# Scalsol/mega.pytorch

Hardware: AMD Instinct MI355X
Metric: frames/sec MEGA R-101 inference, 1000x600 VID clip (higher is better)
Workload: dtype bf16

## Files before the change

mega/pytorch_amd/build.py:

```python
import hashlib
import os
import subprocess
import sys

HERE = os.path.dirname(os.path.abspath(__file__))
CSRC = os.path.join(HERE, "csrc")
LIB = os.path.join(HERE, "libmega_hip.so")
STAMP = os.path.join(HERE, "csrc", ".build_stamp")
SOURCES = {
    "igemm.hip": [],
    "igemm8.hip": [],
    "igemm4.hip": [],
    "igemm2.hip": [],
    "stream1x1.hip": [],
    "spatial.hip": [],
    "boxes.hip": ["-ffp-contract=off"],
    "relation.hip": ["-mllvm", "-amdgpu-mfma-vgpr-form=1"],
    "frames.hip": ["-ffp-contract=off"],
    "fgfa.hip": [],
    "assemble.hip": [],
    "conv64.hip": [],
    "bneck64.hip": [],
    "vid_eval.hip": ["-ffp-contract=off"],
    "seq_nms.hip": ["-ffp-contract=off"],
}
HIPCC = os.environ.get("HIPCC", "/opt/rocm/bin/hipcc")
BASE_FLAGS = ["--offload-arch=gfx950", "-O3", "-std=c++17", "-fPIC", "-Wno-unused-result"]
if os.environ.get("MEGA_BUILD_EXPERIMENTS") == "1":
    BASE_FLAGS.append("-DMEGA_EXPERIMENTS")


def _probe_flags(flags):
    if not flags or not os.path.exists(HIPCC):
        return list(flags)
    import tempfile
    with tempfile.TemporaryDirectory() as td:
        src = os.path.join(td, "probe.hip")
        with open(src, "w") as f:
            f.write("#include <hip/hip_runtime.h>\n__global__ void mega_probe() {}\n")
        cmd = [HIPCC, "--offload-arch=gfx950", "-O1"] + list(flags) + ["-c", src, "-o", os.path.join(td, "probe.o")]
        if subprocess.run(cmd, stdout=subprocess.PIPE, stderr=subprocess.STDOUT).returncode == 0:
            return list(flags)
    sys.stderr.write("build.py: hipcc rejects %s -- building without it\n" % " ".join(flags))
    return []


def _digest():
    h = hashlib.sha256()
    for fn in sorted(os.listdir(CSRC)):
        if fn.endswith((".hip", ".h")):
            h.update(fn.encode())
            h.update(open(os.path.join(CSRC, fn), "rb").read())
    h.update(" ".join(BASE_FLAGS).encode())
    h.update(repr(sorted(SOURCES.items())).encode())
    h.update(open(os.path.abspath(__file__), "rb").read())
    return h.hexdigest()


def build(force=False, verbose=False):
    dig = _digest()
    if not force and os.path.exists(LIB) and os.path.exists(STAMP) and open(STAMP).read().strip() == dig:
        return LIB
    if not os.path.exists(HIPCC):
        if os.path.exists(LIB):
            return LIB
        raise RuntimeError("hipcc not found at %s and no prebuilt %s" % (HIPCC, LIB))
    objs = []
    procs = []
    for src, extra in SOURCES.items():
        path = os.path.join(CSRC, src)
        if not os.path.exists(path):
            continue
        if "-mllvm" in extra:
            extra = _probe_flags(extra)
        obj = os.path.join(CSRC, src.replace(".hip", ".o"))
        cmd = [HIPCC] + BASE_FLAGS + extra + ["-c", path, "-o", obj]
        if verbose:
            print(" ".join(cmd))
        procs.append((src, subprocess.Popen(cmd, stdout=subprocess.PIPE, stderr=subprocess.STDOUT)))
        objs.append(obj)
    for src, pr in procs:
        out, _ = pr.communicate()
        if pr.returncode != 0:
            raise RuntimeError("hipcc failed on %s:\n%s" % (src, out.decode()))
        if verbose and out:
            print(out.decode())
    cmd = [HIPCC, "--offload-arch=gfx950", "-shared", "-fPIC", "-o", LIB] + objs
    subprocess.check_call(cmd)
    with open(STAMP, "w") as f:
        f.write(dig)
    return LIB


if __name__ == "__main__":
    print(build(force="--force" in sys.argv, verbose=True))
```

mega/pytorch_amd/csrc/igemm.hip:

```cpp
#include <cstdio>
#include <cstdlib>

#include "common.h"
#include "igemm_params.h"

namespace {

constexpr int KTB = 128;
constexpr int LDS_STRIDE = 144;
constexpr int NTHREADS = 256;

template <typename T> struct Mma;
template <> struct Mma<bf16_t> {
  __device__ static __forceinline__ void run(f32x16_t& acc, const uint4& a, const uint4& b) {
    bf16x8_t av = __builtin_bit_cast(bf16x8_t, a);
    bf16x8_t bv = __builtin_bit_cast(bf16x8_t, b);
    acc = __builtin_amdgcn_mfma_f32_32x32x16_bf16(av, bv, acc, 0, 0, 0);
  }
};
template <> struct Mma<f16_t> {
  __device__ static __forceinline__ void run(f32x16_t& acc, const uint4& a, const uint4& b) {
    acc = __builtin_amdgcn_mfma_f32_32x32x16_f16(__builtin_bit_cast(f16x8_t, a), __builtin_bit_cast(f16x8_t, b), acc, 0, 0, 0);
  }
};
// ... 235 lines not shown
        asm volatile("" ::: "memory");
#pragma unroll
        for (int it = 0; it < NIT; ++it) {
          const int row = row0 + it * RSTEP;
          float v[OVE];
#pragma unroll
          for (int t = 0; t < OVE; t += 4) {
            const float4 f = *reinterpret_cast<const float4*>(cs + row * CST + cvo + t);
            v[t] = f.x; v[t + 1] = f.y; v[t + 2] = f.z; v[t + 3] = f.w;
          }
          if (HAS_RES) {
            const T* re = reinterpret_cast<const T*>(&rr[i % PD][it]);
#pragma unroll
            for (int t = 0; t < OVE; ++t) v[t] += Elem<T>::ld(re + t);
          }
          u32x4_t o;
          if constexpr (sizeof(OT) == 2) {
#pragma unroll
            for (int d = 0; d < 4; ++d) {
              if constexpr (RELU) {
                const s16x2_t z = {0, 0};
                o[d] = __builtin_bit_cast(unsigned, __builtin_elementwise_max(__builtin_bit_cast(s16x2_t, Half16<OT>::pack2(v[2 * d], v[2 * d + 1])), z));
              } else {
                o[d] = Half16<OT>::pack2(act(v[2 * d]), act(v[2 * d + 1]));
              }
            }
          } else {
#pragma unroll
            for (int t = 0; t < 4; ++t) o[t] = __float_as_uint(RELU ? fmaxf(v[t], 0.f) : act(v[t]));
          }
          __builtin_amdgcn_raw_buffer_store_b128(o, rs_out, out_off(slab_m(i, it)), 0, 0);
        }
        if (HAS_RES && i + PD < TM) ldres(i + PD, rr[i % PD]);
      }
    };
    if (res) {
      if (p.relu == 1) run(std::integral_constant<bool, RES_FAST>{}, std::true_type{});
      else run(std::integral_constant<bool, RES_FAST>{}, std::false_type{});
    } else {
      if (p.relu == 1) run(std::false_type{}, std::true_type{}); else run(std::false_type{}, std::false_type{});
    }
    return;
  }
  if (PS && p.ksplit == 1) return;
#pragma unroll
  for (int i = 0; i < TM; ++i) {
    if (i > 0) __syncthreads();
#pragma unroll
    for (int j = 0; j < TN; ++j) {
      const int nl = wn * WTN + j * 32 + (lane & 31);
      const int rb = wm * 32 + 4 * (lane >> 5);
#pragma unroll
      for (int r = 0; r < 16; ++r) cs[(rb + (r & 3) + 8 * (r >> 2)) * CST + nl] = acc[i][j][r] * sc[j] + bi[j];
    }
    __syncthreads();
    if (p.ksplit > 1) {
      float* part = p.partial + (size_t)blockIdx.z * p.M * p.Cout;
      for (int e = tid; e < 64 * (BN / 4); e += NTHREADS) {
        const int row = e / (BN / 4), cv = e - row * (BN / 4);
        const int m = m0 + (row >> 5) * WTM + i * 32 + (row & 31), n = n0 + cv * 4;
        if (m >= p.M || n >= p.Cout) continue;
        const float4 f = *reinterpret_cast<const float4*>(cs + row * CST + cv * 4);
        if (n + 4 <= p.Cout && p.Cout % 4 == 0) {
          *reinterpret_cast<float4*>(part + (size_t)m * p.Cout + n) = f;
        } else {
          const float v[4] = {f.x, f.y, f.z, f.w};
          for (int t = 0; t < 4 && n + t < p.Cout; ++t) part[(size_t)m * p.Cout + n + t] = v[t];
        }
      }
      continue;
    }
    for (int e = tid; e < 64 * VPR; e += NTHREADS) {
      const int row = e / VPR, cv = e - row * VPR;
      const int m = m0 + (row >> 5) * WTM + i * 32 + (row & 31), n = n0 + cv * OVE;
      if (m >= p.M || n >= p.Cout) continue;
      float v[OVE];
#pragma unroll
      for (int t = 0; t < OVE; t += 4) {
        const float4 f = *reinterpret_cast<const float4*>(cs + row * CST + cv * OVE + t);
        v[t] = f.x; v[t + 1] = f.y; v[t + 2] = f.z; v[t + 3] = f.w;
      }
      if (vec_ok && n + OVE <= p.Cout) {
        if (res) {
          const uint4 rr = *reinterpret_cast<const uint4*>(res + (size_t)m * p.ldr + n);
          const T* re = reinterpret_cast<const T*>(&rr);
#pragma unroll
          for (int t = 0; t < OVE; ++t) v[t] += Elem<T>::ld(re + t);
        }
        uint4 o;
        OT* oe = reinterpret_cast<OT*>(&o);
#pragma unroll
        for (int t = 0; t < OVE; ++t) Elem<OT>::st(oe + t, act(v[t]));
        *reinterpret_cast<uint4*>(out + (size_t)m * p.ldo + n) = o;
      } else {
        for (int t = 0; t < OVE && n + t < p.Cout; ++t) {
          float x = v[t];
          if (res) x += Elem<T>::ld(res + (size_t)m * p.ldr + n + t);
          x = act(x);
          Elem<OT>::st(out + (size_t)m * p.ldo + n + t, x);
        }
      }
    }
  }
}

template <typename T, typename OT, int BM, int BN, bool PS = false>
int launch(const ConvParams& p, hipStream_t st) {
  const int ntm = cdiv(p.M, BM), ntn = cdiv(p.Cout, BN);
  const size_t smem = 2 * (BM + BN) * LDS_STRIDE;
  (void)hipFuncSetAttribute((const void*)igemm_kernel<T, OT, BM, BN, PS>, hipFuncAttributeMaxDynamicSharedMemorySize, (int)smem);
  hipLaunchKernelGGL((igemm_kernel<T, OT, BM, BN, PS>), dim3(ntm * ntn, 1, p.ksplit), dim3(NTHREADS), smem, st, p);
  return mega_check_launch();
}

template <typename T, typename OT>
__global__ __launch_bounds__(256) void splitk_finalize_kernel(ConvParams p) {
  const size_t total = (size_t)p.M * p.Cout;
  const float neg_slope = p.relu == 1 ? 0.f : (p.relu == 2 ? 0.1f : 1.f);
  for (size_t i = (size_t)blockIdx.x * blockDim.x + threadIdx.x; i < total; i += (size_t)gridDim.x * blockDim.x) {
    const int m = (int)(i / p.Cout), n = (int)(i - (size_t)m * p.Cout);
    float v = 0.f;
    for (int z = 0; z < p.ksplit; ++z) v += p.partial[(size_t)z * total + i];
    v = v * (p.scale ? p.scale[n] : 1.f) + (p.bias ? p.bias[n] : 0.f);
    if (p.res) v += Elem<T>::ld((const T*)p.res + (size_t)m * p.ldr + n);
    v = v > 0.f ? v : v * neg_slope;
    if (p.ps) {
      const int HoWo = p.Ho * p.Wo, t = m / HoWo, rem = m - t * HoWo, mh = rem / p.Wo, mw = rem - mh * p.Wo;
      const int q = n / p.ps_C, y = 2 * mh + (q >> 1) - p.ps_crop, x = 2 * mw + (q & 1) - p.ps_crop;
      if ((unsigned)y < (unsigned)p.ps_H && (unsigned)x < (unsigned)p.ps_W)
        Elem<OT>::st((OT*)p.out + ((size_t)(t * p.ps_H + y) * p.ps_W + x) * p.ldo + p.ps_coff + (n - q * p.ps_C), v);
      continue;
    }
    Elem<OT>::st((OT*)p.out + (size_t)m * p.ldo + n, v);
  }
}

template <typename T, typename OT>
int launch_finalize(const ConvParams& p, hipStream_t st) {
  const size_t total = (size_t)p.M * p.Cout;
  const unsigned blocks = (unsigned)((total + 255) / 256 > 8192 ? 8192 : (total + 255) / 256);
  hipLaunchKernelGGL((splitk_finalize_kernel<T, OT>), dim3(blocks), dim3(256), 0, st, p);
  return mega_check_launch();
}

inline int choose_ksplit(int K) { return K >= 32768 ? 3 : 1; }

inline void choose_tile(int M, int Cout, int K, int z, bool bf16, int& kind, int& bm, int& bn) {
  kind = 0;
  const char* force = getenv("MEGA_IGEMM_TILE");
  if (force && sscanf(force, "8:%d", &bm) == 1) { kind = 8; bn = 256; return; }
  if (force && sscanf(force, "4:%d", &bm) == 1) { kind = 4; bn = 256; return; }
  if (force && sscanf(force, "2:%d", &bm) == 1) { kind = 2; bm = 128; bn = 256; return; }
  if (force && sscanf(force, "s:%d", &bm) == 1) { kind = 1; bm = 32; bn = 256; return; }
  if (force && sscanf(force, "%dx%d", &bm, &bn) == 2) return;
  const long b256 = (long)cdiv(M, 256) * cdiv(Cout, 256) * z;
  const long b128 = (long)cdiv(M, 128) * cdiv(Cout, 128) * z;
  const long b12864 = (long)cdiv(M, 128) * cdiv(Cout, 64) * z;
  static const int use8 = getenv("MEGA_IGEMM8") ? atoi(getenv("MEGA_IGEMM8")) : 1;
  static const int min_kt = getenv("MEGA_IGEMM8_MIN_KTILES") ? atoi(getenv("MEGA_IGEMM8_MIN_KTILES")) : 1;
  if (bf16 && use8 && Cout >= 256 && K >= 64 * min_kt) {
    const long t256 = (long)cdiv(M, 256) * cdiv(Cout, 256) * z, t192 = (long)cdiv(M, 192) * cdiv(Cout, 256) * z;
    const long c256 = cdiv((int)t256, 256) * 256L * 8, c192 = cdiv((int)t192, 256) * 192L * 9;
    if (t256 >= 128 || t192 >= 128) {
      kind = 8; bn = 256; bm = c192 < c256 ? 192 : 256;
      return;
    }
  }
  if (K >= 8192 && Cout >= 1024 && b256 >= 700) { bm = 256; bn = 256; }
  else if (Cout > 64 && b128 >= 384) { bm = 128; bn = 128; }
  else if (b12864 >= 384) { bm = 128; bn = 64; }
  else { bm = 64; bn = 64; }
}

template <typename T, typename OT>
int dispatch_tile(const ConvParams& p, hipStream_t st) {
  int kind = 0, bm = 0, bn = 0, rc;
  constexpr bool is_bf16 = sizeof(T) == 2;
  choose_tile(p.M, p.Cout, p.K, p.ksplit, is_bf16, kind, bm, bn);
  if (kind == 8 && !(is_bf16 && mega_igemm8_supports(p))) {
    kind = 0; bm = 128; bn = 128;
  }
  if constexpr (is_bf16 && sizeof(OT) == 2) {
    static const int use_s = getenv("MEGA_STREAM1X1") ? atoi(getenv("MEGA_STREAM1X1")) : 0;
    if ((kind == 1 || (kind == 8 && use_s && !getenv("MEGA_IGEMM_TILE"))) && mega_stream1x1_supports(p, 0))
      return mega_stream1x1_launch(p, Half16<T>::CODE, st);
  }
  if (kind == 1) { kind = is_bf16 && mega_igemm8_supports(p) ? 8 : 0; bm = kind ? 256 : 128; bn = kind ? 256 : 128; }
  if constexpr (is_bf16) {
    static const int use2 = getenv("MEGA_IGEMM2") ? atoi(getenv("MEGA_IGEMM2")) : 0;
    {
      const bool streaming2 = mega_igemm8_streaming(p.R * p.S, p.K) && p.ksplit == 1;
      if (kind == 2 || (kind == 8 && use2 && (use2 > 2 || (streaming2 && (use2 > 1 || p.K <= 128))) && !getenv("MEGA_IGEMM_TILE"))) {
        if (mega_igemm2_supports(p, sizeof(OT) == 4)) return mega_igemm2_launch(p, sizeof(OT) == 4, Half16<T>::CODE, st);
        if (kind == 2) kind = mega_igemm8_supports(p) ? 8 : 0;
        if (kind == 0) { bm = 128; bn = 128; } else if (bm != 192) bm = 256;
      }
    }
    static const int use4 = getenv("MEGA_IGEMM4") ? atoi(getenv("MEGA_IGEMM4")) : 0;
    const bool streaming = mega_igemm8_streaming(p.R * p.S, p.K) && p.ksplit == 1;
    if (kind == 4 || (kind == 8 && use4 && (use4 > 1 || !streaming) && !getenv("MEGA_IGEMM_TILE"))) {
      if (mega_igemm4_supports(p, sizeof(OT) == 4)) {
        rc = mega_igemm4_launch(p, bm == 192 ? 192 : 256, sizeof(OT) == 4, Half16<T>::CODE, st);
        if (rc == MEGA_OK && p.ksplit > 1) rc = launch_finalize<T, OT>(p, st);
        return rc;
      }
      if (kind == 4) kind = mega_igemm8_supports(p) ? 8 : 0;
      if (kind == 0) { bm = 128; bn = 128; }
    }
    if (kind == 8) {
      rc = mega_igemm8_launch(p, bm, sizeof(OT) == 4, Half16<T>::CODE, st);
      if (rc == MEGA_OK && p.ksplit > 1) rc = launch_finalize<T, OT>(p, st);
      return rc;
    }
  }
  if (kind == 8 || kind == 4 || kind == 2) rc = MEGA_ERR_ARG;
  else if (bm == 256 && bn == 256) rc = launch<T, OT, 256, 256>(p, st);
  else if (bm == 256 && bn == 128) rc = launch<T, OT, 256, 128>(p, st);
  else if (bm == 128 && bn == 128) rc = launch<T, OT, 128, 128>(p, st);
  else if (bm == 128 && bn == 64) rc = launch<T, OT, 128, 64>(p, st);
  else rc = launch<T, OT, 64, 64>(p, st);
  if (rc == MEGA_OK && p.ksplit > 1) rc = launch_finalize<T, OT>(p, st);
  return rc;
}

}

static int plan_of(const ConvParams& p, bool bf16_in, bool f32_out) {
  if (bf16_in && !f32_out && !getenv("MEGA_IGEMM_TILE") && mega_conv64_supports(p, 0)) return 6 * 1000000 + 256 * 1000 + 64;
  int kind = 0, bm = 0, bn = 0;
  choose_tile(p.M, p.Cout, p.K, choose_ksplit(p.K), bf16_in, kind, bm, bn);
  if (kind == 1 || kind == 8) {
    static const int use_s = getenv("MEGA_STREAM1X1") ? atoi(getenv("MEGA_STREAM1X1")) : 0;
    ConvParams q = p;
    q.ksplit = choose_ksplit(p.K);
    if (bf16_in && !f32_out && (kind == 1 || (use_s && !getenv("MEGA_IGEMM_TILE"))) && mega_stream1x1_supports(q, 0)) return 1 * 1000000 + 32 * 1000 + 256;
    if (kind == 1) { kind = 8; bm = 256; bn = 256; }
  }
  if (kind == 2 || kind == 8) {
    static const int use2 = getenv("MEGA_IGEMM2") ? atoi(getenv("MEGA_IGEMM2")) : 0;
    ConvParams q = p;
    q.ksplit = choose_ksplit(p.K);
    const bool streaming2 = mega_igemm8_streaming(p.R * p.S, p.K) && q.ksplit == 1;
    if (bf16_in && (kind == 2 || (use2 && (use2 > 2 || (streaming2 && (use2 > 1 || p.K <= 128))) && !getenv("MEGA_IGEMM_TILE"))) && mega_igemm2_supports(q, f32_out))
      return 2 * 1000000 + 128 * 1000 + 256;
    if (kind == 2) { kind = 8; bm = 256; }
  }
  if ((kind == 8 || kind == 4) && !(bf16_in && mega_igemm8_supports(p))) { kind = 0; bm = 128; bn = 128; }
  if (kind == 8 || kind == 4) {
    static const int use4 = getenv("MEGA_IGEMM4") ? atoi(getenv("MEGA_IGEMM4")) : 0;
    const bool streaming = mega_igemm8_streaming(p.R * p.S, p.K) && choose_ksplit(p.K) == 1;
    ConvParams q = p;
    q.ksplit = choose_ksplit(p.K);
    const bool take4 = (kind == 4 || (use4 && (use4 > 1 || !streaming) && !getenv("MEGA_IGEMM_TILE"))) && mega_igemm4_supports(q, f32_out || q.ksplit > 1);
    if (take4) kind = streaming ? 3 : 4;
    else kind = streaming ? 7 : 8;
    if (bm != 192) bm = 256;
  }
  return kind * 1000000 + bm * 1000 + bn;
}

extern "C" int mega_conv2d_nhwc_plan_ex(int N, int H, int W, int Cin, int Cout, int R, int S, int stride, int pad, int dil,
                                        int ldo, int has_residual, int in_dtype, int out_dtype) {
  if (N <= 0 || H <= 0 || W <= 0 || Cin <= 0 || Cout <= 0 || R <= 0 || S <= 0 || stride <= 0 || dil <= 0 || pad < 0) return -1;
  ConvParams p = {};
  p.N = N; p.H = H; p.W = W; p.Cin = Cin; p.Cout = Cout; p.R = R; p.S = S; p.stride = stride; p.pad = pad; p.dil = dil;
  p.Ho = (H + 2 * pad - dil * (R - 1) - 1) / stride + 1;
  p.Wo = (W + 2 * pad - dil * (S - 1) - 1) / stride + 1;
  if (p.Ho <= 0 || p.Wo <= 0) return -1;
  p.M = N * p.Ho * p.Wo;
  p.K = R * S * Cin;
  p.ldo = ldo > 0 ? ldo : Cout;
  p.ldr = p.ldo;
  p.res = has_residual ? (const void*)&p : nullptr;
  p.ksplit = 1;
  const size_t esz = in_dtype == MEGA_F32 ? 4 : 2;
  const size_t ib = (size_t)N * H * W * Cin * esz, wb = (size_t)Cout * p.K * esz;
  p.in_bytes = ib >= 0xFFFFFFF0ull ? 0xFFFFFFF0u : (unsigned)ib;
  p.w_bytes = wb >= 0xFFFFFFF0ull ? 0xFFFFFFF0u : (unsigned)wb;
  return plan_of(p, in_dtype != MEGA_F32, out_dtype == MEGA_F32);
}

extern "C" int mega_conv2d_nhwc_plan(int M, int Cout, int K, int in_dtype) {
  return mega_conv2d_nhwc_plan_ex(M, 1, 1, K, Cout, 1, 1, 1, 0, 1, Cout, 0, in_dtype, in_dtype);
}

extern "C" int mega_conv2d_nhwc_tile(int M, int Cout, int K) { return mega_conv2d_nhwc_plan(M, Cout, K, MEGA_BF16) % 1000000; }

extern "C" size_t mega_conv2d_nhwc_workspace_bytes(int M, int Cout, int K) {
  const int z = choose_ksplit(K);
  return z > 1 ? (size_t)z * M * Cout * sizeof(float) : 0;
}

static int clamp_ksplit(int K, int in_dtype, int want) {
  const int nkt = K / (in_dtype == MEGA_F32 ? 32 : 64);
  int z = want < 1 ? 1 : (want > nkt ? nkt : want);
  while (z > 1 && (z - 1) * cdiv(nkt, z) >= nkt) --z;
  return z < 1 ? 1 : z;
}

extern "C" size_t mega_conv2d_nhwc_ks_workspace_bytes(int M, int Cout, int K, int in_dtype, int ksplit) {
  const int z = clamp_ksplit(K, in_dtype, ksplit);
  return z > 1 ? (size_t)z * M * Cout * sizeof(float) : 0;
}

static int conv2d_impl(const void* in, const void* w, const float* scale, const float* bias,
                       const void* residual, void* out, int N, int H, int W, int Cin, int Cout,
                       int R, int S, int stride, int pad, int dil, int relu, int ldo, int ldr,
                       int in_dtype, int out_dtype, void* ws, size_t ws_bytes, int ksplit, void* stream);

extern "C" int mega_conv2d_nhwc_ws(const void* in, const void* w, const float* scale, const float* bias,
                                   const void* residual, void* out, int N, int H, int W, int Cin, int Cout,
                                   int R, int S, int stride, int pad, int dil, int relu, int ldo, int ldr,
                                   int in_dtype, int out_dtype, void* ws, size_t ws_bytes, void* stream) {
  return conv2d_impl(in, w, scale, bias, residual, out, N, H, W, Cin, Cout, R, S, stride, pad, dil, relu, ldo, ldr, in_dtype,
                     out_dtype, ws, ws_bytes, 0, stream);
}

extern "C" int mega_conv2d_nhwc_ks(const void* in, const void* w, const float* scale, const float* bias,
                                   const void* residual, void* out, int N, int H, int W, int Cin, int Cout,
                                   int R, int S, int stride, int pad, int dil, int relu, int ldo, int ldr,
                                   int in_dtype, int out_dtype, int ksplit, void* ws, size_t ws_bytes, void* stream) {
  if (ksplit < 1) return MEGA_ERR_ARG;
  return conv2d_impl(in, w, scale, bias, residual, out, N, H, W, Cin, Cout, R, S, stride, pad, dil, relu, ldo, ldr, in_dtype,
                     out_dtype, ws, ws_bytes, ksplit, stream);
}

static int conv2d_impl(const void* in, const void* w, const float* scale, const float* bias,
                       const void* residual, void* out, int N, int H, int W, int Cin, int Cout,
                       int R, int S, int stride, int pad, int dil, int relu, int ldo, int ldr,
                       int in_dtype, int out_dtype, void* ws, size_t ws_bytes, int ksplit, void* stream) {
  mega_clear_error();
  if (!in || !w || !out || N <= 0 || H <= 0 || W <= 0 || Cin <= 0 || Cout <= 0 || R <= 0 || S <= 0 || stride <= 0 ||
      dil <= 0 || pad < 0)
    return MEGA_ERR_ARG;
  ConvParams p = {};
  p.in = in; p.w = w; p.scale = scale; p.bias = bias; p.res = residual; p.out = out;
  p.N = N; p.H = H; p.W = W; p.Cin = Cin; p.Cout = Cout; p.R = R; p.S = S;
  p.stride = stride; p.pad = pad; p.dil = dil;
  p.Ho = (H + 2 * pad - dil * (R - 1) - 1) / stride + 1;
  p.Wo = (W + 2 * pad - dil * (S - 1) - 1) / stride + 1;
  if (p.Ho <= 0 || p.Wo <= 0) return MEGA_ERR_ARG;
  p.M = N * p.Ho * p.Wo;
  p.K = R * S * Cin;
  p.ldo = ldo > 0 ? ldo : Cout;
  p.ldr = ldr > 0 ? ldr : Cout;
  p.relu = relu;
  p.ksplit = 1;
  p.partial = nullptr;
  if (ksplit > 0 && in_dtype != MEGA_F32 && in_dtype != MEGA_BF16 && in_dtype != MEGA_F16) return MEGA_ERR_ARG;
  if (ksplit > 0 || ws) {
    const int z = ksplit > 0 ? clamp_ksplit(p.K, in_dtype, ksplit) : choose_ksplit(p.K);
    if (z > 1) {
      if (!ws) return MEGA_ERR_ARG;
      if (ws_bytes < (size_t)z * p.M * Cout * sizeof(float)) return MEGA_ERR_ARG;
      p.ksplit = z;
      p.partial = (float*)ws;
    }
  }
  {
    if (in_dtype != MEGA_F32 && in_dtype != MEGA_BF16 && in_dtype != MEGA_F16) return MEGA_ERR_ARG;
    const size_t esz = in_dtype == MEGA_F32 ? 4 : 2;
    const size_t ib = (size_t)N * H * W * Cin * esz, wb = (size_t)Cout * p.K * esz;
    if (ib >= 0xFFFFFFF0ull || wb >= 0xFFFFFFF0ull) return MEGA_ERR_ARG;
    p.in_bytes = (unsigned)ib;
    p.w_bytes = (unsigned)wb;
  }
  hipStream_t st = (hipStream_t)stream;
  if (in_dtype == MEGA_BF16) {
    if (Cin % 64 != 0) return MEGA_ERR_ARG;
    if (out_dtype == MEGA_BF16 && !getenv("MEGA_IGEMM_TILE") && mega_conv64_supports(p, 0)) return mega_conv64_launch(p, MEGA_BF16, st);
    if (out_dtype == MEGA_BF16) return dispatch_tile<bf16_t, bf16_t>(p, st);
    if (out_dtype == MEGA_F32) return dispatch_tile<bf16_t, float>(p, st);
    return MEGA_ERR_ARG;
  }
  if (in_dtype == MEGA_F16) {
    if (Cin % 64 != 0) return MEGA_ERR_ARG;
    if (out_dtype == MEGA_F16 && !getenv("MEGA_IGEMM_TILE") && mega_conv64_supports(p, 0)) return mega_conv64_launch(p, MEGA_F16, st);
    if (out_dtype == MEGA_F16) return dispatch_tile<f16_t, f16_t>(p, st);
    if (out_dtype == MEGA_F32) return dispatch_tile<f16_t, float>(p, st);
    return MEGA_ERR_ARG;
  }
  if (in_dtype == MEGA_F32) {
    if (Cin % 32 != 0 || out_dtype != MEGA_F32) return MEGA_ERR_ARG;
    return dispatch_tile<float, float>(p, st);
  }
  return MEGA_ERR_ARG;
}

extern "C" int mega_conv2d_nhwc(const void* in, const void* w, const float* scale, const float* bias,
// ... 110 lines not shown
```

mega/pytorch_amd/csrc/igemm_params.h:

```cpp
#pragma once
#include <hip/hip_runtime.h>

struct ConvParams {
  const void* in;
  const void* w;
  const float* scale;
  const float* bias;
  const void* res;
  void* out;
  int N, H, W, Cin, Cout, R, S, stride, pad, dil, Ho, Wo;
  int M, K;
  int ldo, ldr;
  int relu;
  unsigned in_bytes, w_bytes;
  int ksplit;
  float* partial;
  int sp;
  int ldi;
  int kwrap;
  int split_out;
  unsigned mg_howo, sh_howo, mg_wo, sh_wo;
  int ps;
  int ps_H, ps_W, ps_C, ps_crop, ps_coff;
};

int mega_igemm8_launch(const ConvParams& p, int bm, int out_f32, int half_dtype, hipStream_t st);
int mega_igemm8_supports(const ConvParams& p);
int mega_igemm8_streaming(int taps, int K);
int mega_igemm4_supports(const ConvParams& p, int out_f32);
int mega_igemm4_launch(const ConvParams& p, int bm, int out_f32, int half_dtype, hipStream_t st);
int mega_igemm2_supports(const ConvParams& p, int out_f32);
int mega_igemm2_launch(const ConvParams& p, int out_f32, int half_dtype, hipStream_t st);
int mega_stream1x1_supports(const ConvParams& p, int out_f32);
int mega_stream1x1_launch(const ConvParams& p, int half_dtype, hipStream_t st);
int mega_conv64_supports(const ConvParams& p, int out_f32);
int mega_conv64_launch(const ConvParams& p, int half_dtype, hipStream_t st);
```

mega/pytorch_amd/ops.py:

```python
import contextlib
import ctypes
import threading
import math

import torch

from . import _lib

F32, BF16, F16 = 0, 1, 2
_DT = {torch.float32: F32, torch.bfloat16: BF16, torch.float16: F16}
_HALF = (torch.bfloat16, torch.float16)


def _dt(t):
    try:
        return _DT[t.dtype]
    except KeyError:
        raise TypeError("unsupported dtype %s (float32 / bfloat16 / float16 only)" % t.dtype)


_LAUNCH = threading.local()


def _stream():
    s = getattr(_LAUNCH, "s", None)
    return torch.cuda.current_stream().cuda_stream if s is None else s.cuda_stream


@contextlib.contextmanager
def launch_on(stream):
    prev = getattr(_LAUNCH, "s", None)
    _LAUNCH.s = stream if stream is not None else prev
    try:
        yield
    finally:
        _LAUNCH.s = prev


def profiling():
    return _PROF is not None


def _gpu(*ts):
    for t in ts:
        if t is not None and not t.is_cuda:
            raise RuntimeError("mega.pytorch_amd ops need HIP device tensors (no CPU path)")


def _ptr(t):
    return None if t is None else t.data_ptr()


def _ws(nbytes, device):
    return torch.empty(int(nbytes), dtype=torch.uint8, device=device)


class Profiler(object):

    def __init__(self):
        self.items = []

    def begin(self, family, flops=0.0, nbytes=0.0, detail=None):
        e0 = torch.cuda.Event(enable_timing=True)
        e0.record()
        return [family, float(flops), float(nbytes), e0, detail]

    def end(self, tok):
        e1 = torch.cuda.Event(enable_timing=True)
        e1.record()
        tok.append(e1)
        self.items.append(tok)

    def summary(self, by_detail=False):
        torch.cuda.synchronize()
        out = {}
        for fam, fl, nb, e0, det, e1 in self.items:
            d = out.setdefault((fam, det) if by_detail else fam, {"launches": 0, "ms": 0.0, "flops": 0.0, "bytes": 0.0})
            d["launches"] += 1
            d["ms"] += e0.elapsed_time(e1)
            d["flops"] += fl
            d["bytes"] += nb
        return out


_PROF = None


def set_profiler(p):
    global _PROF
    _PROF = p


def _pb(family, flops=0.0, nbytes=0.0, detail=None):
    return None if _PROF is None else _PROF.begin(family, flops, nbytes, detail)


def _pe(tok):
    if tok is not None:
        _PROF.end(tok)


def _igemm_family(lib, M, Cout, K, dtype, shape=None):
    if shape is not None:
        N, H, W, Cin, R, S, stride, pad, dil, ldo, has_res, odt = shape
        t = lib.mega_conv2d_nhwc_plan_ex(N, H, W, Cin, Cout, R, S, stride, pad, dil, ldo, int(has_res), _DT[dtype], _DT[odt])
    else:
        t = lib.mega_conv2d_nhwc_plan(M, Cout, K, _DT[dtype])
    kind, t = t // 1000000, t % 1000000
    if kind == 6:
        return "conv64_bf16_3x3"
    f32out = shape is not None and dtype in _HALF and (shape[-1] == torch.float32 or (kind in (2, 3, 4, 7, 8) and lib.mega_conv2d_nhwc_workspace_bytes(M, Cout, K) > 0))
    return "igemm%s_%s_%dx%d%s" % ({8: "8", 7: "8s", 4: "4", 3: "4s", 2: "2", 1: "s"}.get(kind, ""), {torch.bfloat16: "bf16", torch.float16: "f16"}.get(dtype, "f32"),
                                   t // 1000, t % 1000, "_f32out" if f32out else "")


def conv2d_nhwc(x, w, scale=None, bias=None, residual=None, stride=1, pad=0, dil=1, relu=False, out_dtype=None,
                out=None, ksplit=None):
    _gpu(x, w, scale, bias, residual)
    lib = _lib.load()
    N, H, W, Cin = x.shape
    Cout, R, S, Cin2 = w.shape
    assert Cin == Cin2 and x.is_contiguous() and w.is_contiguous() and x.dtype == w.dtype
    Ho = (H + 2 * pad - dil * (R - 1) - 1) // stride + 1
    Wo = (W + 2 * pad - dil * (S - 1) - 1) // stride + 1
    odt = x.dtype if out_dtype is None else out_dtype
    if out is None:
        out = torch.empty((N, Ho, Wo, Cout), dtype=odt, device=x.device)
    else:
        assert out.dtype == odt and out.shape == (N, Ho, Wo, Cout) and out.is_contiguous()
    if residual is not None:
        assert residual.shape == out.shape and residual.dtype == x.dtype and residual.is_contiguous()
    for v in (scale, bias):
        assert v is None or (v.dtype == torch.float32 and v.numel() == Cout and v.is_contiguous())
    _tok = None
    if _PROF is not None:
        _tok = _pb(_igemm_family(lib, N * Ho * Wo, Cout, R * S * Cin, x.dtype,
                                 (N, H, W, Cin, R, S, stride, pad, dil, Cout, residual is not None, odt)),
                   2.0 * N * Ho * Wo * Cout * R * S * Cin,
                   x.numel() * x.element_size() + w.numel() * w.element_size() + out.numel() * out.element_size()
                   + (0 if residual is None else residual.numel() * residual.element_size()),
                   detail="%dx%dx%d (%dx%d)" % (N * Ho * Wo, Cout, R * S * Cin, R, S))
    if x.numel() * x.element_size() >= 0x7FF00000 or w.numel() * w.element_size() >= 0x7FF00000:
        raise ValueError("conv2d_nhwc: operand of %.2f GiB; the kernels use 32-bit buffer offsets (< 2 GiB per operand): "
                         "lower the frame-stage batch (ClipEngine steps_per_batch) or split the call over M"
                         % (max(x.numel() * x.element_size(), w.numel() * w.element_size()) / 2.0 ** 30))
    if ksplit is not None:
        nb = lib.mega_conv2d_nhwc_ks_workspace_bytes(N * Ho * Wo, Cout, R * S * Cin, _dt(x), int(ksplit))
        ws = _ws(nb, x.device) if nb else None
        rc = lib.mega_conv2d_nhwc_ks(_ptr(x), _ptr(w), _ptr(scale), _ptr(bias), _ptr(residual), _ptr(out), N, H, W, Cin,
                                     Cout, R, S, stride, pad, dil, int(relu), Cout, Cout, _dt(x), _DT[odt], int(ksplit),
                                     _ptr(ws), nb, _stream())
        _pe(_tok)
        _lib.check(rc, "mega_conv2d_nhwc_ks")
        return out
    nb = lib.mega_conv2d_nhwc_workspace_bytes(N * Ho * Wo, Cout, R * S * Cin)
    ws = _ws(nb, x.device) if nb else None
    rc = lib.mega_conv2d_nhwc_ws(_ptr(x), _ptr(w), _ptr(scale), _ptr(bias), _ptr(residual), _ptr(out), N, H, W, Cin,
                                 Cout, R, S, stride, pad, dil, int(relu), Cout, Cout, _dt(x), _DT[odt], _ptr(ws), nb,
                                 _stream())
    _pe(_tok)
    _lib.check(rc, "mega_conv2d_nhwc")
    return out


def pack_deconv4x4s2(wt, dtype, cin_mult):
    Cin, C = wt.shape[:2]
    cp = (Cin + cin_mult - 1) // cin_mult * cin_mult
    w4 = torch.zeros((2, 2, C, 2, 2, cp), dtype=torch.float32)
    wf = wt.detach().float().cpu()
    for a in range(2):
        for b in range(2):
            for r in range(2):
                for s_ in range(2):
                    w4[a, b, :, r, s_, :Cin] = wf[:, :, a + 2 * (1 - r), b + 2 * (1 - s_)].t()
    return w4.view(4 * C, 2, 2, cp).to(dtype).contiguous()


def deconv4x4s2_into(x, w4, bias4, out, coff, relu=0, ksplit=1):
    _gpu(x, w4, bias4, out)
    lib = _lib.load()
    N, H, W, Cin = x.shape
    C = w4.shape[0] // 4
    assert tuple(w4.shape) == (4 * C, 2, 2, Cin) and x.is_contiguous() and w4.is_contiguous() and out.is_contiguous()
    assert x.dtype == w4.dtype == out.dtype and out.shape[0] == N
    H2, W2, ldo = out.shape[1:]
    crop = 0 if (2 * H + 2, 2 * W + 2) == (H2, W2) else 1
    assert H2 + crop <= 2 * H + 2 and W2 + crop <= 2 * W + 2
    M = N * (H + 1) * (W + 1)
    _tok = _pb("deconv_subpixel", 2.0 * M * 4 * C * 4 * Cin, (x.numel() + w4.numel() + N * H2 * W2 * C) * x.element_size(),
               detail="%dx%dx%d (2x2 sub-pixel)" % (M, 4 * C, 4 * Cin))
    nb = lib.mega_conv2d_nhwc_ks_workspace_bytes(M, 4 * C, 4 * Cin, _dt(x), int(ksplit))
    ws = _ws(nb, x.device) if nb else None
    rc = lib.mega_conv2d_nhwc_subpixel(_ptr(x), _ptr(w4), _ptr(bias4), _ptr(out), N, H, W, Cin, C, int(relu), H2, W2, crop, ldo,
                                       coff, _dt(x), int(ksplit), _ptr(ws), nb, _stream())
    _pe(_tok)
    _lib.check(rc, "mega_conv2d_nhwc_subpixel")
    return out


def flow_conv1_combine(ab, bias, dtype, key=None, order=None, T=None, out=None, nwin=0):
    _gpu(ab, bias, order)
    lib = _lib.load()
    S, h, w, c = ab.shape
    if nwin > 0:
        assert order is not None and order.dim() == 2 and order.shape[1] == nwin + 1
        T = order.shape[0] * nwin
    else:
        T = S if T is None else T
        assert T <= S
    assert c == 128 and ab.dtype == torch.float32 and ab.is_contiguous() and bias.dtype == torch.float32 and bias.numel() == 64
    assert dtype in _HALF and (key is not None or order is not None)
    assert order is None or (order.dtype == torch.int32 and order.is_contiguous())
    if out is None:
        out = torch.empty((T, h, w, 64), dtype=dtype, device=ab.device)
    assert out.dtype == dtype and tuple(out.shape) == (T, h, w, 64) and out.is_contiguous()
    _tok = _pb("flow_conv1_combine", 0.0, T * h * w * 64 * 6.0)
    rc = lib.mega_flow_conv1_combine(_ptr(ab), _ptr(bias), _ptr(order), -1 if key is None else int(key), _ptr(out), T, h * w,
                                     int(nwin), _DT[dtype], _stream())
    _pe(_tok)
    _lib.check(rc, "mega_flow_conv1_combine")
    return out


def flow_pred_finish(z, bias, scale, out_dtype):
    _gpu(z, bias)
    lib = _lib.load()
    N, H, W, ldz = z.shape
    assert z.dtype == torch.float32 and z.is_contiguous() and bias.dtype == torch.float32 and bias.numel() == 2
    out = torch.empty((N, H, W, 2), dtype=out_dtype, device=z.device)
    _tok = _pb("flow_pred_finish", 0.0, N * H * W * (18 * 4.0 + 2 * out.element_size()))
    rc = lib.mega_flow_pred_finish(_ptr(z), ldz, _ptr(bias), float(scale), _ptr(out), N, H, W, _DT[out_dtype], _stream())
    _pe(_tok)
    _lib.check(rc, "mega_flow_pred_finish")
    return out


def flow_level_assemble(skip, flow, w_up, b_up, out, C):
    _gpu(skip, flow, w_up, b_up, out)
    lib = _lib.load()
    N, H2, W2, Cs = skip.shape
    _, h, w, two = flow.shape
    assert two == 2 and out.shape[:3] == skip.shape[:3] and flow.shape[0] == N
    assert skip.is_contiguous() and flow.is_contiguous() and out.is_contiguous() and skip.dtype == flow.dtype == out.dtype
    assert w_up.dtype == torch.float32 and tuple(w_up.shape) == (2, 2, 4, 4) and w_up.is_contiguous() and b_up.dtype == torch.float32
    crop = 0 if (2 * h + 2, 2 * w + 2) == (H2, W2) else 1
    _tok = _pb("flow_level_assemble", 0.0, (skip.numel() + N * H2 * W2 * (out.shape[3] - C)) * skip.element_size())
    rc = lib.mega_flow_level_assemble(_ptr(skip), _ptr(flow), _ptr(w_up), _ptr(b_up), _ptr(out), N, H2, W2, Cs, C, out.shape[3],
                                      h, w, crop, _dt(skip), _stream())
    _pe(_tok)
    _lib.check(rc, "mega_flow_level_assemble")
    return out


def bottleneck64(x, w1, s1, b1, w2, s2, b2, w3, s3, b3):
    _gpu(x, w1, s1, b1, w2, s2, b2, w3, s3, b3)
    lib = _lib.load()
    N, H, W, C = x.shape
    assert C == 256 and x.dtype in _HALF and x.is_contiguous()
    assert tuple(w1.shape) == (64, 1, 1, 256) and tuple(w2.shape) == (64, 3, 3, 64) and tuple(w3.shape) == (256, 1, 1, 64)
    for t in (w1, w2, w3):
        assert t.dtype == x.dtype and t.is_contiguous()
    for v, n in ((s1, 64), (b1, 64), (s2, 64), (b2, 64), (s3, 256), (b3, 256)):
        assert v.dtype == torch.float32 and v.numel() == n and v.is_contiguous()
    if x.numel() * 2 >= 0x7FF00000:
        raise ValueError("bottleneck64: operand of %.2f GiB; 32-bit buffer offsets (< 2 GiB)" % (x.numel() * 2 / 2.0 ** 30))
# ... 910 lines not shown
```

Baseline: 885.6.

## Add persistent row-streaming 1x1 conv kernel for K=128 bf16 convolutions

Adds a new persistent kernel for 1x1 stride-1 convolutions with K=128/256. It keeps the full weight slab resident in LDS and lets each wave stream 32-row activation tiles via buffer-to-LDS loads, with the next tile's load issued during the epilogue. The dispatcher routes large-M K=128 bf16 1x1 convs (the igemm8 streaming case) to it by default. The aim is to avoid refetching weights per tile and to overlap loads with MFMA work. In exchange it runs a fixed 256-block grid with one block per CU, which risks low occupancy.

```diff
diff --git a/mega/pytorch_amd/build.py b/mega/pytorch_amd/build.py
--- a/mega/pytorch_amd/build.py
+++ b/mega/pytorch_amd/build.py
@@ -13,6 +13,7 @@
     "igemm4.hip": [],
     "igemm2.hip": [],
     "stream1x1.hip": [],
+    "stream_rows.hip": [],
     "spatial.hip": [],
     "boxes.hip": ["-ffp-contract=off"],
     "relation.hip": ["-mllvm", "-amdgpu-mfma-vgpr-form=1"],
diff --git a/mega/pytorch_amd/csrc/igemm.hip b/mega/pytorch_amd/csrc/igemm.hip
--- a/mega/pytorch_amd/csrc/igemm.hip
+++ b/mega/pytorch_amd/csrc/igemm.hip
@@ -411,6 +411,7 @@
   if (force && sscanf(force, "4:%d", &bm) == 1) { kind = 4; bn = 256; return; }
   if (force && sscanf(force, "2:%d", &bm) == 1) { kind = 2; bm = 128; bn = 256; return; }
   if (force && sscanf(force, "s:%d", &bm) == 1) { kind = 1; bm = 32; bn = 256; return; }
+  if (force && sscanf(force, "r:%d", &bm) == 1) { kind = 5; bm = 32; bn = 128; return; }
   if (force && sscanf(force, "%dx%d", &bm, &bn) == 2) return;
   const long b256 = (long)cdiv(M, 256) * cdiv(Cout, 256) * z;
   const long b128 = (long)cdiv(M, 128) * cdiv(Cout, 128) * z;
@@ -431,6 +432,14 @@
   else { bm = 64; bn = 64; }
 }
 
+inline bool stream_rows_policy(const ConvParams& p, int kind) {
+  if (kind == 5) return true;
+  if (kind != 8 || getenv("MEGA_IGEMM_TILE")) return false;
+  const char* e = getenv("MEGA_STREAM_ROWS");
+  if (e && atoi(e) == 0) return false;
+  return mega_igemm8_streaming(p.R * p.S, p.K) && p.ksplit == 1 && p.K == 128 && p.stride == 1 && p.M >= 20 * 75 * 125;
+}
+
 template <typename T, typename OT>
 int dispatch_tile(const ConvParams& p, hipStream_t st) {
   int kind = 0, bm = 0, bn = 0, rc;
@@ -443,8 +452,10 @@
     static const int use_s = getenv("MEGA_STREAM1X1") ? atoi(getenv("MEGA_STREAM1X1")) : 0;
     if ((kind == 1 || (kind == 8 && use_s && !getenv("MEGA_IGEMM_TILE"))) && mega_stream1x1_supports(p, 0))
       return mega_stream1x1_launch(p, Half16<T>::CODE, st);
-  }
-  if (kind == 1) { kind = is_bf16 && mega_igemm8_supports(p) ? 8 : 0; bm = kind ? 256 : 128; bn = kind ? 256 : 128; }
+    if (stream_rows_policy(p, kind) && mega_stream_rows_supports(p, 0) && mega_stream_rows_aligned(p))
+      return mega_stream_rows_launch(p, Half16<T>::CODE, st);
+  }
+  if (kind == 1 || kind == 5) { kind = is_bf16 && mega_igemm8_supports(p) ? 8 : 0; bm = kind ? 256 : 128; bn = kind ? 256 : 128; }
   if constexpr (is_bf16) {
     static const int use2 = getenv("MEGA_IGEMM2") ? atoi(getenv("MEGA_IGEMM2")) : 0;
     {
@@ -494,6 +505,12 @@
     q.ksplit = choose_ksplit(p.K);
     if (bf16_in && !f32_out && (kind == 1 || (use_s && !getenv("MEGA_IGEMM_TILE"))) && mega_stream1x1_supports(q, 0)) return 1 * 1000000 + 32 * 1000 + 256;
     if (kind == 1) { kind = 8; bm = 256; bn = 256; }
+  }
+  if (kind == 5 || kind == 8) {
+    ConvParams q = p;
+    q.ksplit = choose_ksplit(p.K);
+    if (bf16_in && !f32_out && stream_rows_policy(q, kind) && mega_stream_rows_supports(q, 0)) return 5 * 1000000 + 32 * 1000 + 128;
+    if (kind == 5) { kind = 8; bm = 256; bn = 256; }
   }
   if (kind == 2 || kind == 8) {
     static const int use2 = getenv("MEGA_IGEMM2") ? atoi(getenv("MEGA_IGEMM2")) : 0;
diff --git a/mega/pytorch_amd/csrc/igemm_params.h b/mega/pytorch_amd/csrc/igemm_params.h
--- a/mega/pytorch_amd/csrc/igemm_params.h
+++ b/mega/pytorch_amd/csrc/igemm_params.h
@@ -33,5 +33,8 @@
 int mega_igemm2_launch(const ConvParams& p, int out_f32, int half_dtype, hipStream_t st);
 int mega_stream1x1_supports(const ConvParams& p, int out_f32);
 int mega_stream1x1_launch(const ConvParams& p, int half_dtype, hipStream_t st);
+int mega_stream_rows_supports(const ConvParams& p, int out_f32);
+int mega_stream_rows_aligned(const ConvParams& p);
+int mega_stream_rows_launch(const ConvParams& p, int half_dtype, hipStream_t st);
 int mega_conv64_supports(const ConvParams& p, int out_f32);
 int mega_conv64_launch(const ConvParams& p, int half_dtype, hipStream_t st);
diff --git a/mega/pytorch_amd/csrc/stream_rows.hip b/mega/pytorch_amd/csrc/stream_rows.hip
--- /dev/null
+++ b/mega/pytorch_amd/csrc/stream_rows.hip
@@ -0,0 +1,294 @@
+#include <cstdio>
+#include <cstdlib>
+#include <type_traits>
+
+#include "common.h"
+#include "igemm_params.h"
+
+namespace {
+
+constexpr int NTR = 256;
+__host__ __device__ constexpr int bn_of(int) { return 128; }
+constexpr unsigned OOBR = 0x80000000u;
+
+typedef __attribute__((address_space(3))) void* lds_ptr_r;
+typedef unsigned int u32x2r_t __attribute__((ext_vector_type(2)));
+
+__device__ __forceinline__ int rdiv(int n, unsigned mg, unsigned sh) {
+  return (int)((__umulhi((unsigned)n, mg) + (unsigned)n) >> sh);
+}
+
+#define SR_WAIT_VM(n) asm volatile("s_waitcnt vmcnt(%0)" ::"n"(n) : "memory")
+#define SR_WAIT_LDS()                                 \
+  do {                                                \
+    asm volatile("s_waitcnt lgkmcnt(0)" ::: "memory"); \
+    __builtin_amdgcn_sched_barrier(0);                \
+  } while (0)
+
+template <typename HT, int K, bool HAS_RES, bool RELU>
+__global__ __launch_bounds__(NTR, 1) void stream_rows_kernel(ConvParams p) {
+  constexpr int BNR = bn_of(K);
+  constexpr int SLAB = 32 * BNR * 2;
+  constexpr int CPS = BNR / 8;
+  constexpr int RPS = 1024 / (BNR * 2);
+  constexpr int RB = K * 2;
+  constexpr int CPR = K / 8;
+  constexpr int RPI = 1024 / RB;
+  constexpr int NQA = 32 / RPI;
+  constexpr int NQS = SLAB / 1024;
+  constexpr int NKS = K / 16;
+  constexpr int NJ = BNR / 32;
+  constexpr int WLDS = BNR * RB;
+  constexpr int SA = 32 * RB;
+  static_assert(K == 128 || K == 256, "the LDS budget is laid out for K = 128 / 256");
+  static_assert(WLDS + 4 * (SA + SLAB) <= 160 * 1024, "LDS");
+  extern __shared__ __attribute__((aligned(16))) unsigned char smem[];
+
+  const int tid = threadIdx.x;
+  const int lane = tid & 63;
+  const int wave = __builtin_amdgcn_readfirstlane(tid >> 6);
+  const int l31 = lane & 31, h = lane >> 5, sw = l31 & 15;
+
+  const int ntn = p.Cout / BNR;
+  const int xcd = blockIdx.x & 7, loc = blockIdx.x >> 3, per = gridDim.x >> 3;
+  const int tile_n = loc % ntn, grp = loc / ntn, ngrp = per / ntn;
+  const int n0 = tile_n * BNR;
+
+  {
+    const unsigned char* wsrc = reinterpret_cast<const unsigned char*>(p.w) + (size_t)n0 * RB;
+    for (int e = tid; e < BNR * CPR; e += NTR) {
+      const int n = e / CPR, c = e % CPR;
+      const uint4 v = *reinterpret_cast<const uint4*>(wsrc + (size_t)n * RB + c * 16);
+      *reinterpret_cast<uint4*>(smem + n * RB + ((c ^ (n & 15)) * 16)) = v;
+    }
+  }
+  f32x4_t sv[NJ][4], bv[NJ][4];
+  {
+    const bool al16 = ((reinterpret_cast<size_t>(p.scale) | reinterpret_cast<size_t>(p.bias)) & 15) == 0;
+#pragma unroll
+    for (int j = 0; j < NJ; ++j)
+#pragma unroll
+      for (int g = 0; g < 4; ++g) {
+        const int c = n0 + 32 * j + 8 * g + 4 * h;
+        f32x4_t s4 = {1.f, 1.f, 1.f, 1.f}, b4 = {0.f, 0.f, 0.f, 0.f};
+        if (al16) {
+          if (p.scale) s4 = *reinterpret_cast<const f32x4_t*>(p.scale + c);
+          if (p.bias) b4 = *reinterpret_cast<const f32x4_t*>(p.bias + c);
+        } else {
+#pragma unroll
+          for (int u = 0; u < 4; ++u) {
+            if (p.scale) s4[u] = p.scale[c + u];
+            if (p.bias) b4[u] = p.bias[c + u];
+          }
+        }
+        sv[j][g] = s4;
+        bv[j][g] = b4;
+      }
+  }
+  __syncthreads();
+
+  const __amdgpu_buffer_rsrc_t rs_in = __builtin_amdgcn_make_buffer_rsrc(const_cast<void*>(p.in), 0, (int)p.in_bytes, 0x00020000);
+  const __amdgpu_buffer_rsrc_t rs_out = __builtin_amdgcn_make_buffer_rsrc(
+      p.out, 0, (int)(((size_t)(p.M - 1) * p.ldo + p.Cout) * 2), 0x00020000);
+  const __amdgpu_buffer_rsrc_t rs_res = __builtin_amdgcn_make_buffer_rsrc(
+      const_cast<void*>(HAS_RES ? p.res : p.out), 0, HAS_RES ? (int)(((size_t)(p.M - 1) * p.ldr + p.Cout) * 2) : 0, 0x00020000);
+  const float neg_slope = p.relu == 1 ? 0.f : (p.relu == 2 ? 0.1f : 1.f);
+  auto act = [&](float x) { return x > 0.f ? x : x * neg_slope; };
+
+  const unsigned abase = (unsigned)(WLDS + wave * (SA + SLAB));
+  const unsigned sbase = abase + (unsigned)SA;
+  unsigned char* const a_lds = smem + abase;
+  unsigned char* const s_lds = smem + sbase;
+  const unsigned brd = (unsigned)(l31 * RB) + (unsigned)((h ^ sw) * 16);
+  const unsigned ard = abase + brd;
+  const unsigned sep = sbase + (unsigned)(l31 * (BNR * 2)) + (unsigned)(8 * h);
+  const int ssw = l31 & (CPS - 1);
+  const int srow = lane / CPS, spc = lane % CPS;
+  const unsigned srd = sbase + (unsigned)(lane * 16);
+
+  const int T = (p.M + 31) >> 5;
+  const int t_lo = (int)((long long)T * xcd >> 3), t_hi = (int)((long long)T * (xcd + 1) >> 3);
+  const int wid = grp * 4 + wave, nw = ngrp * 4;
+  const int HoWo = p.Ho * p.Wo;
+
+  auto issue_a = [&](int t, bool live) {
+    const int pc = lane % CPR;
+#pragma unroll
+    for (int q = 0; q < NQA; ++q) {
+      const int r = q * RPI + lane / CPR;
+      const int m = t * 32 + r;
+      unsigned off = OOBR;
+      if (live && m < p.M) {
+        const int nimg = rdiv(m, p.mg_howo, p.sh_howo);
+        const int rem = m - nimg * HoWo;
+        const int ho = rdiv(rem, p.mg_wo, p.sh_wo);
+        const int wo = rem - ho * p.Wo;
+        const unsigned pix = (unsigned)((nimg * p.H + ho * p.stride) * p.W + wo * p.stride);
+        off = pix * (unsigned)RB + (unsigned)((pc ^ (r & 15)) * 16);
+      }
+      __builtin_amdgcn_raw_ptr_buffer_load_lds(rs_in, (lds_ptr_r)(a_lds + q * 1024), 16, off, 0, 0, 0);
+    }
+  };
+  auto issue_res = [&](int t, bool live) {
+#pragma unroll
+    for (int q = 0; q < NQS; ++q) {
+      const int r = q * RPS + srow;
+      const int m = t * 32 + r;
+      const unsigned off = live && m < p.M ? ((unsigned)m * (unsigned)p.ldr + (unsigned)n0) * 2u + (unsigned)((spc ^ (r & (CPS - 1))) * 16) : OOBR;
+      __builtin_amdgcn_raw_ptr_buffer_load_lds(rs_res, (lds_ptr_r)(s_lds + q * 1024), 16, off, 0, 0, 0);
+    }
+  };
+
+  int t = t_lo + wid;
+  issue_a(t, t < t_hi);
+  if constexpr (HAS_RES) issue_res(t, t < t_hi);
+  bool first = true;
+  for (; t < t_hi; t += nw) {
+    if (first) {
+      if constexpr (HAS_RES) SR_WAIT_VM(NQS); else SR_WAIT_VM(0);
+    } else {
+      if constexpr (HAS_RES) SR_WAIT_VM(2 * NQS); else SR_WAIT_VM(NQS);
+    }
+    first = false;
+    __builtin_amdgcn_sched_barrier(0);
+
+    f32x16_t acc[NJ];
+#pragma unroll
+    for (int j = 0; j < NJ; ++j)
+#pragma unroll
+      for (int r = 0; r < 16; ++r) acc[j][r] = 0.f;
+
+    u32x4_t fa[2], fb[2][NJ];
+#define SR_RD(ks_, bf_)                                                                       \
+  do {                                                                                        \
+    const unsigned ao = ard ^ (unsigned)(32 * (ks_)), bo = brd ^ (unsigned)(32 * (ks_));      \
+    asm volatile("ds_read_b128 %0, %1" : "=v"(fa[bf_]) : "v"(ao) : "memory");               \
+    _Pragma("unroll") for (int j = 0; j < NJ; ++j) {                                          \
+      const unsigned bj = bo + (unsigned)(j * 32 * RB);                                       \
+      asm volatile("ds_read_b128 %0, %1" : "=v"(fb[bf_][j]) : "v"(bj) : "memory");           \
+    }                                                                                         \
+  } while (0)
+    SR_RD(0, 0);
+#pragma unroll
+    for (int ks = 0; ks < NKS; ++ks) {
+      const int bf = ks & 1;
+      SR_WAIT_LDS();
+      if (ks + 1 < NKS) SR_RD(ks + 1, bf ^ 1);
+#pragma unroll
+      for (int j = 0; j < NJ; ++j) acc[j] = Half16<HT>::mfma32(fb[bf][j], fa[bf], acc[j]);
+      __builtin_amdgcn_sched_barrier(0);
+    }
+#undef SR_RD
+
+    issue_a(t + nw, t + nw < t_hi);
+
+    if constexpr (HAS_RES) SR_WAIT_VM(NQA);
+    __builtin_amdgcn_sched_barrier(0);
+    u32x2r_t rr[NJ][4];
+    if constexpr (HAS_RES) {
+#pragma unroll
+      for (int j = 0; j < NJ; ++j)
+#pragma unroll
+        for (int g = 0; g < 4; ++g) {
+          const unsigned a = sep + (unsigned)((((4 * j + g) ^ ssw)) * 16);
+          asm volatile("ds_read_b64 %0, %1" : "=v"(rr[j][g]) : "v"(a) : "memory");
+        }
+      SR_WAIT_LDS();
+    }
+#pragma unroll
+    for (int j = 0; j < NJ; ++j)
+#pragma unroll
+      for (int g = 0; g < 4; ++g) {
+        float v[4];
+#pragma unroll
+        for (int i = 0; i < 4; ++i) v[i] = fmaf(acc[j][4 * g + i], sv[j][g][i], bv[j][g][i]);
+        if constexpr (HAS_RES) {
+          const u32x2r_t r2 = rr[j][g];
+          v[0] += Half16<HT>::lo(r2[0]); v[1] += Half16<HT>::hi(r2[0]);
+          v[2] += Half16<HT>::lo(r2[1]); v[3] += Half16<HT>::hi(r2[1]);
+        }
+        u32x2r_t o;
+#pragma unroll
+        for (int d = 0; d < 2; ++d) {
+          if constexpr (RELU) {
+            const s16x2_t z = {0, 0};
+            o[d] = __builtin_bit_cast(unsigned, __builtin_elementwise_max(__builtin_bit_cast(s16x2_t, Half16<HT>::pack2(v[2 * d], v[2 * d + 1])), z));
+          } else {
+            o[d] = Half16<HT>::pack2(act(v[2 * d]), act(v[2 * d + 1]));
+          }
+        }
+        const unsigned a = sep + (unsigned)((((4 * j + g) ^ ssw)) * 16);
+        asm volatile("ds_write_b64 %0, %1" ::"v"(a), "v"(o) : "memory");
+      }
+    SR_WAIT_LDS();
+    u32x4_t ov[NQS];
+#pragma unroll
+    for (int q = 0; q < NQS; ++q) {
+      const unsigned a = srd + (unsigned)(q * 1024);
+      asm volatile("ds_read_b128 %0, %1" : "=v"(ov[q]) : "v"(a) : "memory");
+    }
+    SR_WAIT_LDS();
+#pragma unroll
+    for (int q = 0; q < NQS; ++q) {
+      const int r = q * RPS + srow;
+      const int m = t * 32 + r;
+      const unsigned off = m < p.M ? ((unsigned)m * (unsigned)p.ldo + (unsigned)n0) * 2u + (unsigned)((spc ^ (r & (CPS - 1))) * 16) : OOBR;
+      __builtin_amdgcn_raw_buffer_store_b128(ov[q], rs_out, off, 0, 0);
+    }
+    __builtin_amdgcn_sched_barrier(0);
+    if constexpr (HAS_RES) issue_res(t + nw, t + nw < t_hi);
+  }
+  SR_WAIT_VM(0);
+}
+
+#undef SR_WAIT_VM
+#undef SR_WAIT_LDS
+
+inline void magic_div_r(int d, unsigned& mg, unsigned& sh) {
+  sh = 0;
+  while ((1ull << sh) < (unsigned long long)d) ++sh;
+  mg = (unsigned)((((1ull << sh) - (unsigned long long)d) << 32) / (unsigned long long)d + 1ull);
+}
+
+template <typename HT, int K>
+int launch_r(const ConvParams& p0, hipStream_t st) {
+  ConvParams p = p0;
+  magic_div_r(p.Ho * p.Wo, p.mg_howo, p.sh_howo);
+  magic_div_r(p.Wo, p.mg_wo, p.sh_wo);
+  const int lds = bn_of(K) * K * 2 + 4 * (32 * K * 2 + 32 * bn_of(K) * 2);
+  const int grid = 256;
+  auto go = [&](auto kern) {
+    (void)hipFuncSetAttribute((const void*)kern, hipFuncAttributeMaxDynamicSharedMemorySize, lds);
+    hipLaunchKernelGGL(kern, dim3(grid), dim3(NTR), lds, st, p);
+    return mega_check_launch();
+  };
+  if (p.res) return p.relu == 1 ? go(stream_rows_kernel<HT, K, true, true>) : go(stream_rows_kernel<HT, K, true, false>);
+  return p.relu == 1 ? go(stream_rows_kernel<HT, K, false, true>) : go(stream_rows_kernel<HT, K, false, false>);
+}
+
+}
+
+int mega_stream_rows_supports(const ConvParams& p, int out_f32) {
+  if (p.sp || p.ps || p.ksplit != 1 || out_f32) return 0;
+  if (p.R != 1 || p.S != 1 || p.pad != 0 || p.K != p.Cin) return 0;
+  if (p.K != 128 && p.K != 256) return 0;
+  if (p.Cout % bn_of(p.K) != 0 || 32 % (p.Cout / bn_of(p.K)) != 0) return 0;
+  if (p.M <= 0 || p.ldo % 8 != 0 || p.ldo < p.Cout || (p.res && (p.ldr % 8 != 0 || p.ldr < p.Cout))) return 0;
+  if (p.in_bytes >= 0x7FF00000u || (size_t)p.N * p.H * p.W * p.Cin * 2 > (size_t)p.in_bytes) return 0;
+  if (((size_t)(p.M - 1) * p.ldo + p.Cout) * 2 >= 0x7FF00000ull) return 0;
+  if (p.res && ((size_t)(p.M - 1) * p.ldr + p.Cout) * 2 >= 0x7FF00000ull) return 0;
+  return 1;
+}
+
+int mega_stream_rows_aligned(const ConvParams& p) {
+  return ((reinterpret_cast<size_t>(p.w) | reinterpret_cast<size_t>(p.in) | reinterpret_cast<size_t>(p.out) |
+           reinterpret_cast<size_t>(p.res)) & 15) == 0 &&
+         ((reinterpret_cast<size_t>(p.scale) | reinterpret_cast<size_t>(p.bias)) & 3) == 0;
+}
+
+int mega_stream_rows_launch(const ConvParams& p, int half_dtype, hipStream_t st) {
+  if (!mega_stream_rows_supports(p, 0) || !mega_stream_rows_aligned(p)) return MEGA_ERR_ARG;
+  if (half_dtype == MEGA_F16) return p.K == 256 ? launch_r<f16_t, 256>(p, st) : launch_r<f16_t, 128>(p, st);
+  if (half_dtype == MEGA_BF16) return p.K == 256 ? launch_r<bf16_t, 256>(p, st) : launch_r<bf16_t, 128>(p, st);
+  return MEGA_ERR_ARG;
+}
diff --git a/mega/pytorch_amd/ops.py b/mega/pytorch_amd/ops.py
--- a/mega/pytorch_amd/ops.py
+++ b/mega/pytorch_amd/ops.py
@@ -110,7 +110,7 @@
     if kind == 6:
         return "conv64_bf16_3x3"
     f32out = shape is not None and dtype in _HALF and (shape[-1] == torch.float32 or (kind in (2, 3, 4, 7, 8) and lib.mega_conv2d_nhwc_workspace_bytes(M, Cout, K) > 0))
-    return "igemm%s_%s_%dx%d%s" % ({8: "8", 7: "8s", 4: "4", 3: "4s", 2: "2", 1: "s"}.get(kind, ""), {torch.bfloat16: "bf16", torch.float16: "f16"}.get(dtype, "f32"),
+    return "igemm%s_%s_%dx%d%s" % ({8: "8", 7: "8s", 5: "r", 4: "4", 3: "4s", 2: "2", 1: "s"}.get(kind, ""), {torch.bfloat16: "bf16", torch.float16: "f16"}.get(dtype, "f32"),
                                    t // 1000, t % 1000, "_f32out" if f32out else "")
 
 
```

Result: no change. 879.7, median of 2 (-0.7%).
